# emonosuke/emoASR

Measured on AMD Instinct MI355X. Metric: train frames/sec + decode RTF, Conformer-CTC 23M, 80-mel, 1/2/4/8 GPU, higher is better.
Workload: dtype bf16; 1 GPU; CTC(Conformer) 23M `L2`, bf16, SpecAugment on-GPU, synthetic LibriSpeech-shaped batches (2000 utts, lognormal lengths, ASRBatchSampler packing 30000 frames/50 utts per GPU), one step = accum_grad 5 micro-batches (the reference's accum_grad: 5, asr/train_asr.py:106-128, stacked through the engine in one pass) fwd+bwd, then all-reduce+clip+Adam; dropout 0.1; accum_grad=5, stacked_micro_batches=True, parallelism=dp1

## Files before the change

emoasr_amd/csrc/ctc.hip:

```cpp
#include <algorithm>
#include "common.h"
#include "../../include/emoasr_hip.h"

namespace {

__device__ __forceinline__ float lat_add(float a, float b) {
  const float m = fmaxf(a, b);
  if (m == -INFINITY) return -INFINITY;
  return m + __logf(1.f + __expf(-fabsf(a - b)));
}
__device__ __forceinline__ float lat_add3(float a, float b, float c) {
  const float m = fmaxf(a, fmaxf(b, c));
  if (m == -INFINITY) return -INFINITY;
  return m + __logf(__expf(a - m) + __expf(b - m) + __expf(c - m));
}

template <typename T>
__global__ __launch_bounds__(256) void row_lse_kernel(int V, const T* __restrict__ logits, long ld,
                                                      float* __restrict__ lse, int aligned) {
  __shared__ float red[16];
  const T* row = logits + (long)blockIdx.x * ld;
  constexpr int VEC = 16 / sizeof(T);
  float m = -INFINITY, s = 0.f;
  const int nv = aligned ? V / VEC : 0;
  for (int i = threadIdx.x; i < nv; i += 256) {
    const Vec16<T> v = load16(row + (long)i * VEC);
    float lm = v.get(0);
#pragma unroll
    for (int j = 1; j < VEC; ++j) lm = fmaxf(lm, v.get(j));
    if (lm > m) { s *= __expf(m - lm); m = lm; }
    if (m == -INFINITY) continue;
#pragma unroll
    for (int j = 0; j < VEC; ++j) s += __expf(v.get(j) - m);
  }
  for (int i = nv * VEC + threadIdx.x; i < V; i += 256) {
    const float x = to_f32(row[i]);
    if (x > m) { s *= __expf(m - x); m = x; }
    if (m != -INFINITY) s += __expf(x - m);
  }
  const float gm = block_max(m, red);
  const float gs = block_sum(m == -INFINITY ? 0.f : s * __expf(m - gm), red);
  if (threadIdx.x == 0) lse[blockIdx.x] = gm + logf(gs);
}

__device__ __forceinline__ int ext_label(const int* lab, int s, int blank) {
  return (s & 1) ? lab[s >> 1] : blank;
}

struct UttRows { const long* row0; const int* tpad; const float* uscale; };

template <typename T>
__global__ __launch_bounds__(256) void ctc_gather_kernel(int Tn, int S, int Lmax, const T* __restrict__ logits,
                                                         long ld, const float* __restrict__ lse,
// ... 109 lines not shown
                                                       T* __restrict__ grad, long ldg, const UttRows ur, int aligned) {
  extern __shared__ float rowbuf[];
  const int b = blockIdx.y, t = blockIdx.x;
  if (ur.tpad && t >= ur.tpad[b]) return;
  const long row = (long)b * Tn + t;
  const long lrow = ur.row0 ? ur.row0[b] + t : row;
  T* g = grad + lrow * ldg;
  const float nl = nll[b];
  const bool vec = aligned && (V % 8 == 0) && (ld % 8 == 0) && (ldg % 8 == 0);
  if (t >= elens[b] || !isfinite(nl)) {
    if (vec) {
      float z[8] = {0.f, 0.f, 0.f, 0.f, 0.f, 0.f, 0.f, 0.f};
      for (int v = threadIdx.x * 8; v < V; v += 2048) store8<T>(g + v, z);
    } else {
      for (int v = threadIdx.x; v < V; v += 256) g[v] = from_f32<T>(0.f);
    }
    return;
  }
  const float l = lse[lrow];
  const T* lg = logits + lrow * ld;
  if (vec) {
    for (int v = threadIdx.x * 8; v < V; v += 2048) {
      float x[8];
      load8<T>(lg + v, x);
#pragma unroll
      for (int e = 0; e < 8; ++e) rowbuf[v + e] = __expf(x[e] - l);
    }
  } else {
    for (int v = threadIdx.x; v < V; v += 256) rowbuf[v] = __expf(to_f32(lg[v]) - l);
  }
  __syncthreads();
  const int Sb = 2 * ylens[b] + 1;
  const int* lab = labels + (long)b * Lmax;
  for (int s = threadIdx.x; s < Sb; s += 256) {
    const long o = row * S + s;
    const float occ = __expf(alpha[o] + beta[o] - lp[o] + nl);
    if (occ > 0.f) atomicAdd(&rowbuf[ext_label(lab, s, blank)], -occ);
  }
  __syncthreads();
  const float gs = (gscale_dev ? gscale * gscale_dev[0] : gscale) * (ur.uscale ? ur.uscale[b] : 1.f);
  if (vec) {
    for (int v = threadIdx.x * 8; v < V; v += 2048) {
      float x[8];
#pragma unroll
      for (int e = 0; e < 8; ++e) x[e] = rowbuf[v + e] * gs;
      store8<T>(g + v, x);
    }
  } else {
    for (int v = threadIdx.x; v < V; v += 256) g[v] = from_f32<T>(rowbuf[v] * gs);
  }
}

template <typename T>
__global__ __launch_bounds__(256) void argmax_kernel(int V, const T* __restrict__ logits, long ld,
                                                     int* __restrict__ best) {
  __shared__ float rv[4];
  __shared__ int ri[4];
  const T* row = logits + (long)blockIdx.x * ld;
  float m = -INFINITY; int mi = 0x7fffffff;
  for (int v = threadIdx.x; v < V; v += 256) {
    const float x = to_f32(row[v]);
    if (x > m || (x == m && v < mi)) { m = x; mi = v; }
  }
#pragma unroll
  for (int o = 32; o > 0; o >>= 1) {
    const float om = __shfl_xor(m, o, 64);
    const int oi = __shfl_xor(mi, o, 64);
    if (om > m || (om == m && oi < mi)) { m = om; mi = oi; }
  }
  if ((threadIdx.x & 63) == 0) { rv[threadIdx.x >> 6] = m; ri[threadIdx.x >> 6] = mi; }
  __syncthreads();
  if (threadIdx.x == 0) {
    for (int w = 1; w < 4; ++w)
      if (rv[w] > m || (rv[w] == m && ri[w] < mi)) { m = rv[w]; mi = ri[w]; }
    best[blockIdx.x] = mi == 0x7fffffff ? 0 : mi;
  }
}

__global__ __launch_bounds__(64) void collapse_kernel(int B, int Tn, const int* __restrict__ best, const int* __restrict__ elens,
                                                      int blank, int* __restrict__ hyp, int* __restrict__ hyplen) {
  const int b = blockIdx.x, lane = threadIdx.x;
  if (b >= B) return;
  const int len = min(elens[b], Tn);
  int n = 0, carry = -1;
  for (int t0 = 0; t0 < len; t0 += 64) {
    const int t = t0 + lane;
    const int v = t < len ? best[(long)b * Tn + t] : blank;
    int prev = __shfl_up(v, 1, 64);
    if (lane == 0) prev = carry;
    const bool keep = t < len && v != prev && v != blank;
    const unsigned long long mask = __ballot(keep);
    if (keep) hyp[(long)b * Tn + n + __popcll(mask & ((1ull << lane) - 1ull))] = v;
    n += __popcll(mask);
    carry = __shfl(v, 63, 64);
  }
  if (lane == 0) hyplen[b] = n;
}

}

extern "C" int emoasr_row_lse(int dtype, int M, int V, const void* logits, long ld, float* lse,
                              void* stream) {
  if (M == 0) return 0;
  const int vec = dtype == EMO_BF16 ? 8 : 4;
  const int aligned = (ld % vec == 0) && (((uintptr_t)logits & 15) == 0);
  EMO_DISPATCH(dtype, (row_lse_kernel<T><<<M, 256, 0, (hipStream_t)stream>>>(V, (const T*)logits, ld, lse,
// ... 13 lines not shown
extern "C" int emoasr_ctc_forward_rows(int dtype, int B, int Tn, int V, int Lmax, const void* logits, long ld,
                                       const float* lse, const int* labels, const int* elens, const int* ylens,
                                       int blank, const long* row0, float* lp, float* alpha, float* beta, float* nll,
                                       void* stream) {
  const int S = 2 * Lmax + 1;
  const UttRows ur{row0, nullptr, nullptr};
  EMO_CHECK(S <= 1024, "ctc: 2*Lmax+1=%d exceeds 1024 lattice states", S);
  if (B == 0 || Tn == 0) return 0;
  hipStream_t s = (hipStream_t)stream;
  dim3 ggrid(Tn, B);
  const int gthreads = std::min(256, cdiv(S, 64) * 64);
  EMO_DISPATCH(dtype, (ctc_gather_kernel<T><<<ggrid, gthreads, 0, s>>>(Tn, S, Lmax, (const T*)logits, ld, lse,
                                                                      labels, elens, ylens, blank, lp, ur)));
  const int threads = cdiv(S, 64) * 64;
  ctc_lattice_kernel<<<2 * B, threads, sizeof(float) * 2 * (S + 4), s>>>(B, Tn, S, Lmax, lp, labels, elens,
                                                                        ylens, blank, alpha, beta, nll);
  EMO_LAUNCH_CHECK();
  return 0;
}

extern "C" int emoasr_ctc_grad(int dtype, int B, int Tn, int V, int Lmax, const void* logits, long ld,
                               const float* lse, const int* labels, const int* elens, const int* ylens,
                               int blank, const float* lp, const float* alpha, const float* beta,
                               const float* nll, float gscale, const float* gscale_dev, void* grad, long ldg,
                               void* stream) {
  return emoasr_ctc_grad_rows(dtype, B, Tn, V, Lmax, logits, ld, lse, labels, elens, ylens, blank, lp, alpha, beta, nll, gscale,
                              gscale_dev, nullptr, nullptr, nullptr, grad, ldg, stream);
}

extern "C" int emoasr_ctc_grad_rows(int dtype, int B, int Tn, int V, int Lmax, const void* logits, long ld,
                                    const float* lse, const int* labels, const int* elens, const int* ylens,
                                    int blank, const float* lp, const float* alpha, const float* beta,
                                    const float* nll, float gscale, const float* gscale_dev, const long* row0, const int* tpad,
                                    const float* uscale, void* grad, long ldg, void* stream) {
  const int S = 2 * Lmax + 1;
  EMO_CHECK((row0 != nullptr) == (tpad != nullptr), "ctc_grad_rows: row0 and tpad go together");
  const UttRows ur{row0, tpad, uscale};
  EMO_CHECK((size_t)V * 4 <= 160 * 1024 - 256, "ctc_grad: V=%d too large for an LDS row", V);
  if (B == 0 || Tn == 0) return 0;
  dim3 grid(Tn, B);
  const int aligned = (((uintptr_t)logits | (uintptr_t)grad) & 15) == 0;
  EMO_DISPATCH(dtype, {
    if ((size_t)V * 4 > 64 * 1024)
      hipFuncSetAttribute((const void*)ctc_grad_kernel<T>, hipFuncAttributeMaxDynamicSharedMemorySize, V * 4);
    ctc_grad_kernel<T><<<grid, 256, sizeof(float) * V, (hipStream_t)stream>>>(
        Tn, V, S, Lmax, (const T*)logits, ld, lse, labels, elens, ylens, blank, lp, alpha, beta, nll, gscale,
        gscale_dev,
        (T*)grad, ldg, ur, aligned);
  });
  EMO_LAUNCH_CHECK();
  return 0;
}

extern "C" int emoasr_ctc_greedy(int dtype, int B, int Tn, int V, const void* logits, long ld,
                                 const int* elens, int blank, int* best, int* hyp, int* hyplen,
                                 void* stream) {
  if (B == 0 || Tn == 0) return 0;
  hipStream_t s = (hipStream_t)stream;
  EMO_DISPATCH(dtype, (argmax_kernel<T><<<B * Tn, 256, 0, s>>>(V, (const T*)logits, ld, best)));
  collapse_kernel<<<B, 64, 0, s>>>(B, Tn, best, elens, blank, hyp, hyplen);
  EMO_LAUNCH_CHECK();
  return 0;
}
```

emoasr_amd/engine/encoder.py:

```python
import math
import os

import torch

from .. import ops
from ..ops import ACT_RELU, ACT_SWISH
from .arena import AttnStash, ConvStash, FFNStash, LayerRecord, ParamArena, _Stash, _cfg, h2d_i32, h2d_pack, sinusoid
from .las import LASDecoder
from .rnn_encoder import RNNEncoder
from .rnnt import RNNTDecoder
from .transformer_decoder import TransformerDecoder


class CTCEngine(TransformerDecoder, RNNTDecoder, RNNEncoder, LASDecoder):

    def __init__(self, cfg, module, compute_dtype=torch.bfloat16, bn_buffers=None, f32_split=False, arena=None):
        self.cfg = cfg
        self.split = bool(f32_split) and compute_dtype == torch.float32
        self.d = cfg.enc_hidden_size
        self.h = _cfg(cfg, "enc_num_attention_heads", 0)
        self.nl = cfg.enc_num_layers
        self.conformer = cfg.encoder_type == "conformer"
        self.rnn_enc = cfg.encoder_type == "rnn"
        self.rel = _cfg(cfg, "pos_encode_type", "abs") == "rel"
# ... 467 lines not shown

    def encoder_backward_stacked(self, st, deouts):
        self._defer_wgrads = self._group_wgrads
        try:
            with self._scope():
                self._encoder_bwd_stacked(st, deouts)
        finally:
            self._defer_wgrads = False
            self._wq = []
            self._ln_deferred = []

    def _ctc_train_stacked(self, batches, blank, scales, head):
        A = self.arena
        n = len(batches)
        scales = [1.0 / n] * n if scales is None else [float(v) for v in scales]
        dev = batches[0][0].device
        segs_h, rows_h = [], [0]
        for xs, _, _, _ in batches:
            Bk, Tk, Fd = xs.shape
            T1 = (Tk - 3) // 2 + 1
            segs_h.append((Bk, (T1 - 3) // 2 + 1))
            rows_h.append(rows_h[-1] + Bk * segs_h[-1][1])
        elens_h = [((int(v) - 1) // 2 - 1) // 2 for b in batches for v in b[1]]
        ylens_all = [int(v) for _, _, _, yl in batches for v in yl]
        Lmax = max(max(ylens_all), 1)
        lab = torch.zeros(sum(b for b, _ in segs_h), Lmax, dtype=torch.int32)
        row0, tpad, uscale, b0 = [], [], [], 0
        segw = torch.zeros(n, sum(b for b, _ in segs_h), dtype=torch.float32)
        for k, (_, _, ys, ylens) in enumerate(batches):
            B, T2 = segs_h[k]
            yk = torch.as_tensor(ys)[:, :Lmax].to(torch.int32)
            lab[b0:b0 + B, : yk.shape[1]] = yk
            row0 += [rows_h[k] + b * T2 for b in range(B)]
            tpad += [T2] * B
            uscale += [scales[k] / B] * B
            segw[k, b0:b0 + B] = 1.0 / B
            b0 += B
        elens_d, labels, yl, row0_d, tpad_d, uscale_d, segw_d = h2d_pack(
            [torch.tensor(elens_h, dtype=torch.int32), lab, torch.tensor(ylens_all, dtype=torch.int32),
             torch.tensor(row0, dtype=torch.int64), torch.tensor(tpad, dtype=torch.int32),
             torch.tensor(uscale, dtype=torch.float32), segw], dev)
        eouts, st = self._encoder_fwd_stacked([b[0] for b in batches], [b[1] for b in batches], elens_dev=elens_d)
        segs, rows, elens, Btot, Tmax = st.segs, st.rows, st.elens, st.Btot, st.Tmax
        assert list(segs) == segs_h and list(rows) == rows_h
        w = A.w(head + ".weight")
        V = w.shape[0]
        assert V % 8 == 0, "ctc_train_stacked: vocabulary must be a multiple of 8"
        logits, lse = ops.gemm_nt_lse(eouts, w, A.p(head + ".bias"))
        Vp = (V + 63) // 64 * 64
        dlp = torch.empty(logits.shape[0], Vp, device=dev, dtype=logits.dtype)
        if Vp > V:
            dlp[:, V:].zero_()
        dlogits = dlp[:, :V]
        lp, alpha, beta, nll = ops.ctc_forward_rows(logits, lse, labels, elens, yl, blank, row0_d, Tmax)
        losses = (segw_d * torch.nan_to_num(nll, nan=0.0, posinf=0.0, neginf=0.0)).sum(1)
        ops.ctc_grad_rows(logits, lse, labels, elens, yl, blank, lp, alpha, beta, nll, 1.0, row0_d, tpad_d, uscale_d, dlogits)
        if self.dtype == torch.bfloat16 and os.environ.get("EMOASR_HEAD_NT", "1") != "0":
            self._wgrad(dlogits, eouts, A.g(head + ".weight", tuple(w.shape)), 1.0, A.g(head + ".bias"), 1.0)
            w_t = torch.zeros(w.shape[1], Vp, device=dev, dtype=w.dtype)
            w_t[:, :V].copy_(w.t())
            deouts = ops.gemm_nt(dlp, w_t)
        else:
            deouts = self._lin_bwd(dlogits, eouts, head + ".weight", head + ".bias")
        if self.grad_hook is not None:
            self._flush_wgrads()
            self.grad_hook(A.offsets[head + ".weight"])
        self._encoder_bwd_stacked(st, deouts)
        return losses

    def _lin_bwd(self, dy, x_in, wname, bname, alpha=1.0, **epi):
        A = self.arena
        w = A.w(wname)
        w2 = w.view(w.shape[0], -1)
        self._wgrad(dy, x_in, A.g(wname, tuple(w2.shape)), alpha, A.g(bname), alpha)
        return ops.gemm_nn(dy, w2, alpha=alpha, **epi)

    def _wgrad(self, dy, x_in, out, alpha=1.0, colsum=None, colsum_scale=1.0):
        if self._defer_wgrads:
            self._wq.append((dy, x_in, out, alpha, colsum, colsum_scale))
        else:
            ops.gemm_tn(dy, x_in, out=out, alpha=alpha, accumulate=True, colsum=colsum, colsum_scale=colsum_scale)

    def _hook_after_layer(self, li):
        if not self._layer_rt.wgrad_side:
            self.grad_hook(self._layer_offset(li))
            return
        self._layer_rt.join_wgrads(keep=1)
        if li + 1 < self.nl:
            self.grad_hook(self._layer_offset(li + 1))

    def _layer_offset(self, li):
        if self._layer_lo is None:
            lo = {}
            for n, o in self.arena.offsets.items():
                if n.startswith("encoder.transformers."):
                    k = int(n.split(".")[2])
                    lo[k] = min(lo.get(k, o), o)
            self._layer_lo = lo
        return self._layer_lo[li]

    def _flush_wgrads(self):
        if not self._wq:
            return
        if self._side_wgrads:
            main = torch.cuda.current_stream()
            if self._side is None:
                self._side = torch.cuda.Stream(device=main.device)
            ev = torch.cuda.Event()
            ev.record(main)
            self._side.wait_event(ev)
            ops.gemm_tn_grouped(self._wq, stream=self._side.cuda_stream)
            self._inflight.append(self._wq)
        else:
# ... 255 lines not shown
```

emoasr_amd/lib.py:

```python
import contextlib
import ctypes
import os
from ctypes import (POINTER, Structure, c_char_p, c_float, c_int, c_long, c_uint64,
                    c_void_p)

_HERE = os.path.dirname(os.path.abspath(__file__))
LIB_PATH = os.environ.get("EMOASR_HIP_LIB") or os.path.join(_HERE, "libemoasr_hip.so")

F32, BF16, F32X3 = 0, 1, 2
ACT_NONE, ACT_RELU, ACT_SWISH, ACT_GELU = 0, 1, 2, 3


class Epilogue(Structure):
    _fields_ = [("bias", c_void_p), ("residual", c_void_p), ("pre_out", c_void_p),
                ("dact_pre", c_void_p), ("alpha", c_float), ("res_scale", c_float),
                ("act", c_int), ("dact", c_int), ("ldr", c_int), ("out_f32", c_int),
                ("drop_p", c_float), ("seed", c_uint64)]


class AttnArgs(Structure):
    _fields_ = [("B", c_int), ("H", c_int), ("DK", c_int), ("Tq", c_int), ("Tk", c_int),
                ("ldq", c_long), ("ldk", c_long), ("ldv", c_long), ("ldo", c_long), ("ldp", c_long),
                ("q", c_void_p), ("k", c_void_p), ("v", c_void_p), ("pos", c_void_p),
                ("bias_u", c_void_p), ("bias_v", c_void_p), ("klens", c_void_p),
# ... 205 lines not shown
    "emoasr_attn_step": [I, I, I, I, P, P, P, P, P, P],
    "emoasr_joint_beam_step": [I, POINTER(JointStep), P, P],
    "emoasr_joint_beam_step_parts": [I, POINTER(JointStep), I, P],
    "emoasr_joint_beam_graph_build": [I, POINTER(JointStep), I, I, P],
    "emoasr_joint_beam_graph_launch": [I, I, P],
    "emoasr_attn_dropmask": [I, POINTER(AttnArgs), P, I, P],
    "emoasr_attn_fwd": [I, POINTER(AttnArgs), P],
    "emoasr_attn_bwd": [I, POINTER(AttnArgs), P],
    "emoasr_attn_bwd_fused": [I, POINTER(AttnArgs), P, ctypes.c_size_t, P],
    "emoasr_glu_fwd": [I, I, I, P, P, P],
    "emoasr_glu_bwd": [I, I, I, P, P, P, P],
    "emoasr_dwconv_fwd": [I, I, I, I, I, P, P, P, P, P],
    "emoasr_dwconv_bwd_x": [I, I, I, I, I, P, P, P, P],
    "emoasr_dwconv_fwd_stats": [I, I, I, I, I, P, P, P, P, P, P],
    "emoasr_bn_stats_finalize": [I, I, I, P, P, P, P, P, F, P, P],
    "emoasr_dwconv_bwd_w": [I, I, I, I, I, P, P, P, P, I, P, P],
    "emoasr_bn_stats": [I, I, I, P, P, P, P, P, F, P],
    "emoasr_bn_swish_fwd": [I, I, I, P, P, P, P, P, F, P, P],
    "emoasr_bn_swish_bwd": [I, I, I, P, P, P, P, P, P, F, P, P, P, P, P],
    "emoasr_glu_dwconv_fwd": [I, I, I, I, I, P, P, P, P, P, P],
    "emoasr_bn_swish_bwd_sums": [I, I, I, P, P, P, P, P, P, F, P, P, P, P, P],
    "emoasr_conv_bwd_fused": [I, I, I, I, I, P, P, P, P, P, P, F, P, P, P, P, P, P, P, P],
    "emoasr_strided_copy": [I, I, P, P, I, I, I, I, L, L, L, L, I, P],
    "emoasr_transpose_cast_batched": [I, I, P, P],
    "emoasr_scale_dropout": [I, L, P, P, F, F, U64, P],
    "emoasr_posenc": [I, I, I, I, P, P, F, F, U64, P, P],
    "emoasr_add": [I, L, P, P, P, P],
    "emoasr_row_lse": [I, I, I, P, L, P, P],
    "emoasr_gemm_nt_lse": [I, I, I, I, P, L, P, L, P, L, P, P, P, P],
    "emoasr_ctc_forward": [I, I, I, I, I, P, L, P, P, P, P, I, P, P, P, P, P],
    "emoasr_ctc_grad": [I, I, I, I, I, P, L, P, P, P, P, I, P, P, P, P, F, P, P, L, P],
    "emoasr_rnnt_greedy": [I, I, I, I, I, I, I, I, I, P, P, P, P, P, P, P, P, P, P, P, P, P, L, P, P, P, P],
    "emoasr_wgrad_side_join": [I, P],
    "emoasr_rnnt_beam_lstm": [I, I, I, I, P, L, P, P, P, P, P, P, P, P, P, P, I, P],
    "emoasr_rnnt_beam_joint": [I, I, I, I, I, P, P, P, P, P, P, P, P],
    "emoasr_rnnt_beam_pick": [I, I, I, I, I, P, L, P, L, P],
    "emoasr_rnnlm_step": [I, I, I, I, I, I, I, P, P, P, P, P, P, P, P, P, P, P, P, L, I, P, P, L, P],
    "emoasr_las_attend_fwd": [I, POINTER(LasAttend), P],
    "emoasr_las_attend_bwd": [I, POINTER(LasAttend), P],
    "emoasr_las_dropmask": [POINTER(LasAttend), P, P],
    "emoasr_mlm_expand": [I, I, I, P, P, P, I, I, I, I, P, P, P, P, P],
    "emoasr_sample_rows": [I, I, I, P, L, P, P, U64, L, P, P, P, P],
    "emoasr_gumbel_noise": [I, I, U64, L, P, L, P],
    "emoasr_electra_corrupt": [I, I, P, P, P, P, P, P, P, P],
    "emoasr_bce_head_fwd": [I, I, I, P, L, P, P, P, P, P, P, P, P],
    "emoasr_bce_head_bwd": [I, I, I, P, L, P, P, P, P, F, P, P, L, P, P, P],
    "emoasr_ctc_token_conf": [I, I, I, I, P, L, P, P, P, I, P, P, P, P],
    "emoasr_correct_fuse": [I, I, I, I, I, I, P, L, P, P, L, P, L, F, P, P, P],
    "emoasr_edit_align": [I, I, I, I, P, P, P, P, P, I, P, P, P, P, P, P, P, P],
    "emoasr_rescore_grid": [I, I, I, I, P, P, P, P, P, P, P, P, P, P],
    "emoasr_ctc_beam_batch": [I, I, I, I, P, L, P, P, I, I, ctypes.c_double, I, P, P, P, P, P, L, P, P],
    "emoasr_ctc_forward_rows": [I, I, I, I, I, P, L, P, P, P, P, I, P, P, P, P, P, P],
    "emoasr_ctc_grad_rows": [I, I, I, I, I, P, L, P, P, P, P, I, P, P, P, P, F, P, P, P, P, P, L, P],
    "emoasr_ctc_greedy": [I, I, I, I, P, L, P, I, P, P, P, P],
    "emoasr_embed_fwd": [I, I, I, I, P, P, P, F, F, U64, P, P],
    "emoasr_embed_bwd": [I, I, I, P, P, F, F, U64, P, P],
    "emoasr_lsm_loss": [I, I, I, P, L, P, P, F, P, F, P, P, L, P],
    "emoasr_soft_ce": [I, I, I, P, L, P, P, L, P, P, P, P, F, P, F, P, P, L, P],
    "emoasr_ctc_best_path": [I, I, I, P, P, P, P, P, P, I, P, P],
    "emoasr_ctc_label_map": [I, I, P, P, I, I, P, P, P],
    "emoasr_rnnt_best_path": [I, I, I, P, P, P, P, P, P],
    "emoasr_log_softmax": [I, I, I, P, L, P, L, F, P, L, P],
    "emoasr_topk": [I, I, I, P, L, P, L, P, P, P, P],
    "emoasr_ctc_prefix_init": [I, I, P, I, P, P],
    "emoasr_ctc_prefix_score": [I, I, I, I, P, P, I, P, P, P, P, P, P, I, I, P, P, P],
    "emoasr_lstm_cell_fwd": [I, I, I, P, P, P, L, P, P, P],
    "emoasr_lstm_cell_bwd": [I, I, I, P, L, P, P, P, P, P, P, P],
    "emoasr_lstm_seq_fwd": [I, I, I, I, P, P, P, P, P, P, P, P],
    "emoasr_lstm_seq_bwd": [I, I, I, I, P, P, P, P, P, P, P, L, P],
    "emoasr_bilstm_cell_fwd": [I, I, I, I, I, P, P, L, P, P, P, P, P, P, P, P],
    "emoasr_bilstm_cell_bwd": [I, I, I, I, I, P, P, P, P, P, P, P, P, P],
    "emoasr_bilstm_out": [I, I, I, I, P, P, P, P, F, U64, P],
    "emoasr_bilstm_seq_fwd": [I, I, I, I, P, P, L, P, P, P, P, P, P, P],
    "emoasr_bilstm_seq_bwd": [I, I, I, I, P, P, P, P, P, P, P, P, L, P],
    "emoasr_joint_tanh": [I, I, I, I, I, P, P, P, P],
    "emoasr_joint_reduce": [I, I, I, I, I, P, P, P, P],
    "emoasr_rnnt_forward": [I, I, I, I, I, I, P, P, P, P, I, P, P, P, P, P, P, P],
    "emoasr_rnnt_grad": [I, I, I, I, I, I, P, P, P, P, P, P, P, P, P, P, I, F, P, P, P],
    "emoasr_rnnt_head_fwd": [I, L, I, I, I, I, I, I, P, P, P, P, P, I, P, L, P, P, P, P],
    "emoasr_rnnt_ycol": [I, I, I, I, P, P, P, P],
    "emoasr_rnnt_forward_parts": [I, I, I, I, P, P, P, P, P, P, P, P, P, P],
    "emoasr_rnnt_coef": [I, I, I, I, P, P, P, P, P, P, P, P, P, F, P, P, P, P],
    "emoasr_rnnt_head_grad": [I, I, I, I, P, P, P, P, P, I, P, L, P],
    "emoasr_ce_head_fwd": [I, I, I, I, P, P, P, P, P, P, P, P, P, P, P, P],
    "emoasr_ce_head_sample_fwd": [I, I, I, I, P, P, P, P, P, P, P, P, P, P, P, U64, L, P, P],
    "emoasr_ce_head_grad": [I, I, I, I, P, P, P, P, P, P, F, P, P, P, L, P],
    "emoasr_act_bwd": [I, L, I, P, P, P, P],
    "emoasr_argmax_rows": [I, I, I, P, L, P, P],
    "emoasr_first_not_equal": [I, P, I, P, P],
    "emoasr_sqnorm": [L, P, P, P],
    "emoasr_adam_step": [L, P, P, P, P, F, F, F, F, F, I, P, F, F, P],
    "emoasr_adam_step_ex": [L, P, P, P, P, F, F, F, F, F, I, P, F, F, P, P],
    "emoasr_adamw_step": [L, P, P, P, P, F, F, F, F, I, P, F, F, P, P, P, I, P],
    "emoasr_specaug_apply": [I, I, I, P, P, I, I, P, P, P],
    "emoasr_fbank": [P, L, I, I, I, I, F, P, P, P, I, P],
    "emoasr_cmvn": [I, I, P, P, P, P],
}


class EmoasrHipError(RuntimeError):
    pass


_lib = None


# ... 164 lines not shown
```

emoasr_amd/ops.py:

```python
import ctypes
from ctypes import byref, c_void_p

import os
import threading

import torch

from . import lib
from .lib import ACT_GELU, ACT_NONE, ACT_RELU, ACT_SWISH, BF16, F32, F32X3, AttnArgs, Epilogue

_DT = {torch.float32: F32, torch.bfloat16: BF16}


def dt(t):
    if t.dtype == torch.float32 and split_products():
        return F32X3
    return _DT[t.dtype]


def _p(t):
    return None if t is None else c_void_p(t.data_ptr())


_STREAM_CACHE = None
# ... 592 lines not shown
    B, T, V = logits.shape
    Lmax = labels.shape[1]
    S = 2 * Lmax + 1
    dev = logits.device
    lp = torch.empty(B, T, S, device=dev, dtype=torch.float32)
    alpha = torch.empty(B, T, S, device=dev, dtype=torch.float32)
    beta = torch.empty(B, T, S, device=dev, dtype=torch.float32)
    nll = torch.empty(B, device=dev, dtype=torch.float32)
    lib.call("emoasr_ctc_forward", dt(logits), B, T, V, Lmax, _p(logits), logits.stride(1), _p(lse), _p(labels),
             _p(elens), _p(ylens), blank, _p(lp), _p(alpha), _p(beta), _p(nll), _stream())
    return lp, alpha, beta, nll


def ctc_grad(logits, lse, labels, elens, ylens, blank, lp, alpha, beta, nll, gscale, gscale_dev=None, out=None):
    B, T, V = logits.shape
    ld = logits.stride(1)
    if out is not None:
        assert out.shape == logits.shape and out.dtype == logits.dtype and out.stride(2) == 1
        grad = out
    else:
        grad = torch.empty_like(logits) if ld == V else torch.empty(B, T, ld, device=logits.device, dtype=logits.dtype)[..., :V]
    lib.call("emoasr_ctc_grad", dt(logits), B, T, V, labels.shape[1], _p(logits), logits.stride(1), _p(lse),
             _p(labels), _p(elens), _p(ylens), blank, _p(lp), _p(alpha), _p(beta), _p(nll), gscale, _p(gscale_dev),
             _p(grad),
             grad.stride(1), _stream())
    return grad


def ctc_forward_rows(logits2, lse, labels, elens, ylens, blank, row0, Tmax):
    M, V = logits2.shape
    B, Lmax = labels.shape
    S = 2 * Lmax + 1
    dev = logits2.device
    lp = torch.empty(B, Tmax, S, device=dev, dtype=torch.float32)
    alpha = torch.empty(B, Tmax, S, device=dev, dtype=torch.float32)
    beta = torch.empty(B, Tmax, S, device=dev, dtype=torch.float32)
    nll = torch.empty(B, device=dev, dtype=torch.float32)
    assert row0.dtype == torch.int64
    lib.call("emoasr_ctc_forward_rows", dt(logits2), B, Tmax, V, Lmax, _p(logits2), logits2.stride(0), _p(lse), _p(labels),
             _p(elens), _p(ylens), blank, _p(row0), _p(lp), _p(alpha), _p(beta), _p(nll), _stream())
    return lp, alpha, beta, nll


def ctc_grad_rows(logits2, lse, labels, elens, ylens, blank, lp, alpha, beta, nll, gscale, row0, tpad, uscale, out):
    M, V = logits2.shape
    B, Tmax, _ = lp.shape
    assert out.shape == logits2.shape and out.dtype == logits2.dtype and tpad.dtype == torch.int32 and uscale.dtype == torch.float32
    lib.call("emoasr_ctc_grad_rows", dt(logits2), B, Tmax, V, labels.shape[1], _p(logits2), logits2.stride(0), _p(lse), _p(labels),
             _p(elens), _p(ylens), blank, _p(lp), _p(alpha), _p(beta), _p(nll), gscale, None, _p(row0), _p(tpad), _p(uscale),
             _p(out), out.stride(0), _stream())
    return out


def ctc_greedy(logits, elens, blank):
    B, T, V = logits.shape
    dev = logits.device
    buf = torch.empty(2 * B * T + B, device=dev, dtype=torch.int32)
    best, hyp, hyplen = buf[:B * T].view(B, T), buf[B * T:2 * B * T].view(B, T), buf[2 * B * T:]
    lib.call("emoasr_ctc_greedy", dt(logits), B, T, V, _p(logits), logits.stride(1), _p(elens), blank, _p(best),
             _p(hyp), _p(hyplen), _stream())
    return best, hyp, hyplen


def embed_fwd(ids, table, pe, scale, drop_p=0.0, seed=0):
    B, L = ids.shape
    d = table.shape[1]
    out = torch.empty(B, L, d, device=table.device, dtype=table.dtype)
    lib.call("emoasr_embed_fwd", dt(table), B * L, L, d, _p(ids), _p(table), _p(pe), scale, drop_p, seed, _p(out),
             _stream())
    return out


def embed_bwd(ids, dout, scale, dtable, drop_p=0.0, seed=0):
    B, L = ids.shape
    lib.call("emoasr_embed_bwd", dt(dout), B * L, dout.shape[-1], _p(ids), _p(dout), scale, drop_p, seed,
             _p(_chk(dtable, torch.float32)), _stream())


def lsm_loss(logits, labels, w, lsm_prob, want_grad=False, gscale=1.0, gscale_dev=None, grad=None):
    M, V, ld = _rows(_chk(logits))
    loss = torch.empty(M, device=logits.device, dtype=torch.float32)
    if grad is not None:
        assert want_grad and _chk(grad, logits.dtype).shape == logits.shape and grad.stride(1) == 1
    else:
        grad = torch.empty_like(logits) if want_grad else None
    lib.call("emoasr_lsm_loss", dt(logits), M, V, _p(logits), ld, _p(labels), _p(w), lsm_prob, _p(loss), gscale,
             _p(gscale_dev), _p(grad), 0 if grad is None else grad.stride(0), _stream())
    return loss, grad


def mlm_expand(ys, ylens, row0, r_begin, r_count, Np, mask_id, pad_id=0, total=None, out=None):
    B, N = _chk(ys, torch.int32).shape
    assert ys.is_contiguous() and ylens.numel() == B and row0.numel() == B + 1
    _chk(ylens, torch.int32), _chk(row0, torch.int32)
    assert r_begin >= 0 and r_count >= 1 and (total is None or r_begin + r_count <= total), (r_begin, r_count, total)
    if out is None:
        dev = ys.device
        out = (torch.empty(r_count, Np, device=dev, dtype=torch.int32),) + tuple(
            torch.empty(r_count, device=dev, dtype=torch.int32) for _ in range(3))
    ids, klens, idx, labels = out
    for t in out:
        assert _chk(t, torch.int32).is_contiguous() and t.shape[0] >= r_count
    assert ids.shape[1] == Np
    lib.call("emoasr_mlm_expand", B, N, Np, _p(ys), _p(ylens), _p(row0), r_begin, r_count, mask_id, pad_id, _p(ids), _p(klens),
             _p(idx), _p(labels), _stream())
    return ids[:r_count], klens[:r_count], idx[:r_count], labels[:r_count]
# ... 760 lines not shown
```

include/emoasr_hip.h:

```cpp
#ifndef EMOASR_HIP_H
#define EMOASR_HIP_H
#include <stddef.h>
#include <stdint.h>
#ifdef __cplusplus
extern "C" {
#endif

enum { EMOASR_F32 = 0, EMOASR_BF16 = 1, EMOASR_F32X3 = 2 };
enum { EMOASR_ACT_NONE = 0, EMOASR_ACT_RELU = 1, EMOASR_ACT_SWISH = 2,
       EMOASR_DACT_MUL = 6 };
#define EMOASR_ACT_SAVE_DACT 0x100

const char* emoasr_last_error(void);
int emoasr_version(void);
int emoasr_set_option(const char* name, int value);
int emoasr_get_option(const char* name, int* value, int* default_value);
int emoasr_option_count(void);
const char* emoasr_option_name(int index);
int emoasr_timer_read(const char* name, int* calls, double* ms, int reset);
int emoasr_timer_read_ex(const char* name, int* calls, double* ms, double* flops, double* bytes, int reset);

typedef struct {
  const float* bias;
  const void* residual;
// ... 145 lines not shown
int emoasr_dwconv_bwd_w(int dtype, int B, int T, int C, int K, const void* dy, const void* x, float* dw,
                        float* dbias, int accumulate, float* scratch, void* stream);
long emoasr_dwconv_bwd_w_scratch_floats(int B, int T, int C, int K);
int emoasr_bn_stats(int dtype, int M, int C, const void* y, float* mean, float* var,
                    float* running_mean, float* running_var, float momentum, void* stream);
int emoasr_bn_swish_fwd(int dtype, int M, int C, const void* y, const float* mean, const float* var,
                        const float* gamma, const float* beta, float eps, void* z, void* stream);
long emoasr_bn_swish_bwd_scratch_floats(int M, int C);
int emoasr_bn_swish_bwd(int dtype, int M, int C, const void* dz, const void* y, const float* mean,
                        const float* var, const float* gamma, const float* beta, float eps, void* dy,
                        float* dgamma, float* dbeta, float* scratch, void* stream);
int emoasr_glu_dwconv_fwd(int dtype, int B, int Tn, int C, int K, const void* g, const float* w, const float* bias, void* c,
                          float* part, void* stream);
int emoasr_bn_swish_bwd_sums(int dtype, int M, int C, const void* dz, const void* y, const float* mean, const float* var,
                             const float* gamma, const float* beta, float eps, float* dgamma, float* dbeta, float* scratch,
                             float** tot_out, void* stream);
int emoasr_conv_bwd_fused(int dtype, int B, int Tn, int C, int K, const void* ds, const void* cv, const float* mean,
                          const float* var, const float* gamma, const float* beta, float eps, const float* tot, const void* g,
                          const float* w, void* dg, float* dw, float* dbias, float* scratch, void* stream);

int emoasr_strided_copy(int dtype_in, int dtype_out, const void* in, void* out, int d0, int d1, int d2,
                        int d3, long s0, long s1, long s2, long s3, int accumulate, void* stream);
int emoasr_scale_dropout(int dtype, long n, const void* x, void* y, float scale, float drop_p,
                         uint64_t seed, void* stream);
int emoasr_posenc(int dtype, int B, int T, int N, const void* x, const float* pe, float scale,
                  float drop_p, uint64_t seed, void* y, void* stream);
int emoasr_act_bwd(int dtype, long n, int act, const void* dy, const void* pre, void* dx, void* stream);
int emoasr_add(int dtype, long n, const void* a, const void* b, void* y, void* stream);

typedef struct emoasr_tc_item {
  const float* src; void* dst;
  int rows, cols; long ld_dst;
} emoasr_tc_item_t;
#define EMOASR_TC_MAX 64
int emoasr_transpose_cast_batched(int dtype_out, int n, const emoasr_tc_item_t* items, void* stream);

int emoasr_row_lse(int dtype, int M, int V, const void* logits, long ld, float* lse, void* stream);
int emoasr_gemm_nt_lse(int dtype, int M, int N, int K, const void* A, long lda, const void* B, long ldb, void* C, long ldc,
                       const float* bias, float* part, float* lse, void* stream);
int emoasr_ctc_forward(int dtype, int B, int T, int V, int Lmax, const void* logits, long ld,
                       const float* lse, const int* labels, const int* elens, const int* ylens, int blank,
                       float* lp, float* alpha, float* beta, float* nll, void* stream);
int emoasr_ctc_grad(int dtype, int B, int T, int V, int Lmax, const void* logits, long ld,
                    const float* lse, const int* labels, const int* elens, const int* ylens, int blank,
                    const float* lp, const float* alpha, const float* beta, const float* nll,
                    float gscale, const float* gscale_dev, void* grad, long ldg, void* stream);
int emoasr_ctc_forward_rows(int dtype, int B, int Tn, int V, int Lmax, const void* logits, long ld, const float* lse,
                            const int* labels, const int* elens, const int* ylens, int blank, const long* row0, float* lp,
                            float* alpha, float* beta, float* nll, void* stream);
int emoasr_ctc_grad_rows(int dtype, int B, int Tn, int V, int Lmax, const void* logits, long ld, const float* lse,
                         const int* labels, const int* elens, const int* ylens, int blank, const float* lp, const float* alpha,
                         const float* beta, const float* nll, float gscale, const float* gscale_dev, const long* row0,
                         const int* tpad, const float* uscale, void* grad, long ldg, void* stream);
int emoasr_ctc_greedy(int dtype, int B, int T, int V, const void* logits, long ld, const int* elens,
                      int blank, int* best, int* hyp, int* hyplen, void* stream);

int emoasr_embed_fwd(int dtype, int M, int L, int d, const int* ids, const void* table, const float* pe,
                     float scale, float drop_p, uint64_t seed, void* out, void* stream);
int emoasr_embed_bwd(int dtype, int M, int d, const int* ids, const void* dout, float scale, float drop_p,
                     uint64_t seed, float* dtable, void* stream);
int emoasr_lsm_loss(int dtype, int M, int V, const void* logits, long ld, const int* labels, const float* w,
                    float lsm_prob, float* loss, float gscale, const float* gscale_dev, void* grad, long ldg,
                    void* stream);

int emoasr_soft_ce(int dtype, int R, int V, const void* logits, long ld, const int* lrow, const float* soft, long lds,
                   const int* src, const int* hard, const float* w_soft, const float* w_hard, float lsm_prob,
                   float* loss, float gscale, const float* gscale_dev, void* grad, long ldg, void* stream);
int emoasr_ctc_best_path(int B, int Tn, int Lmax, const float* lp, const float* alpha, const float* beta,
                         const int* labels, const int* elens, const int* ylens, int blank, int* aligns, void* stream);
int emoasr_ctc_label_map(int B, int Tn, const int* aligns, const int* xlens, int blank, int position, int* label_map,
                         int* count, void* stream);

int emoasr_rnnt_best_path(int B, int Tn, int U, const float* alpha, const float* beta, const int* elens,
                          const int* ylens, int* aligns, void* stream);

int emoasr_log_softmax(int dtype, int M, int V, const void* x, long ldx, const float* add, long lda, float mu,
                       float* out, long ldo, void* stream);
int emoasr_topk(int M, int V, int k, const float* x, long ldx, const float* aux, long ldaux, float* vals,
                int* idx, float* aux_out, void* stream);
int emoasr_beam_scores_topk(int dtype, int M, int V, int k, const void* dec, long ldd, const float* lm, long ldl, float mu,
                            float* vals, int* idx, float* lm_at, void* stream);
int emoasr_ctc_prefix_init(int T, int V, const float* x, int blank, float* r, void* stream);
int emoasr_ctc_prefix_score(int nb, int T, int V, int cw, const float* x, const float* prev_states, int cw_prev,
                            const int* parent, const int* pcand, const float* init_state, const int* last,
                            const int* out_len, const int* cands, int blank, int eos, float* log_psi,
                            float* states, void* stream);

int emoasr_lstm_cell_fwd(int dtype, int B, int H, const void* gates_pre, const float* c_prev, void* h, long ldh,
                         float* c, void* gates_act, void* stream);
int emoasr_lstm_cell_bwd(int dtype, int B, int H, const void* dh_out, long lddh, const void* dh_rec, float* dc,
                         const void* gates_act, const float* c_prev, const float* c, void* dgates_pre,
                         void* stream);
int emoasr_lstm_seq_supported(int dtype, int B, int H);
int emoasr_lstm_seq_fwd(int dtype, int U, int B, int H, const void* pre, const void* w_hh, const void* h0, const float* c0,
                        void* hseq, float* cseq, void* gact, void* stream);
long emoasr_lstm_seq_bwd_ws_bytes(int B, int H);
int emoasr_lstm_seq_bwd(int dtype, int U, int B, int H, const void* dh_seq, const void* gact, const float* cseq, const float* c0,
                        const void* w_hh, void* dgp, void* ws, long ws_bytes, void* stream);
long emoasr_lstm_coop_status(void);
int emoasr_bilstm_cell_fwd(int dtype, int B, int T, int H, int s, const int* elens, const void* pre, long ldp, const void* rec,
                           void* hstate, float* cstate, void* hseq, void* hprev, float* cseq, void* gact, void* stream);
int emoasr_bilstm_cell_bwd(int dtype, int B, int T, int H, int s, const int* elens, const void* dy, const void* dh_rec,
                           float* dcstate, const void* gact, const float* cseq, void* dg, void* dgc, void* stream);
int emoasr_bilstm_out(int dtype, int B, int T, int H, const int* elens, const void* x0, const void* x1, void* y, float drop_p,
                      uint64_t seed, void* stream);
int emoasr_bilstm_seq_supported(int dtype, int B, int H);
// ... 325 lines not shown
```

Before: 6.184 million frames/s.

## Split CTC gradient into dense softmax pass overlapped with lattice forward plus sparse fix

The CTC gradient is split into two kernels. A dense kernel writes softmax(logits)*scale for every row, and it runs on a side stream at the same time as the alpha/beta lattice forward. A sparse fix kernel then subtracts occupancies only at label and blank columns, writing a value only where the bf16 result differs. This removes the serialized full-vocabulary pass that followed the forward and replaces LDS atomics with per-label accumulation. The cost is extra stream and event management, a different handling of repeated labels, and possible small numerical differences.

Result: no change. 6.199 million frames/s (median of 5 runs) (+0.2%).

```diff
diff --git a/emoasr_amd/csrc/ctc.hip b/emoasr_amd/csrc/ctc.hip
--- a/emoasr_amd/csrc/ctc.hip
+++ b/emoasr_amd/csrc/ctc.hip
@@ -1,4 +1,7 @@
 #include <algorithm>
+#include <map>
+#include <mutex>
+#include <utility>
 #include "common.h"
 #include "../../include/emoasr_hip.h"
 
@@ -214,6 +217,132 @@
 }
 
 template <typename T>
+__global__ __launch_bounds__(256) void ctc_grad_dense_kernel(int Tn, int V, const T* __restrict__ logits, long ld,
+                                                             const float* __restrict__ lse, const int* __restrict__ elens,
+                                                             float gscale, const float* __restrict__ gscale_dev,
+                                                             T* __restrict__ grad, long ldg, const UttRows ur, int aligned) {
+  const int b = blockIdx.y, t = blockIdx.x;
+  if (ur.tpad && t >= ur.tpad[b]) return;
+  const long lrow = ur.row0 ? ur.row0[b] + t : (long)b * Tn + t;
+  T* g = grad + lrow * ldg;
+  const bool vec = aligned && (V % 8 == 0) && (ld % 8 == 0) && (ldg % 8 == 0);
+  if (t >= elens[b]) {
+    if (vec) {
+      float z[8] = {0.f, 0.f, 0.f, 0.f, 0.f, 0.f, 0.f, 0.f};
+      for (int v = threadIdx.x * 8; v < V; v += 2048) store8<T>(g + v, z);
+    } else {
+      for (int v = threadIdx.x; v < V; v += 256) g[v] = from_f32<T>(0.f);
+    }
+    return;
+  }
+  const float l = lse[lrow];
+  const T* lg = logits + lrow * ld;
+  const float gs = (gscale_dev ? gscale * gscale_dev[0] : gscale) * (ur.uscale ? ur.uscale[b] : 1.f);
+  if (vec) {
+    for (int v = threadIdx.x * 8; v < V; v += 2048) {
+      float x[8];
+      load8<T>(lg + v, x);
+#pragma unroll
+      for (int e = 0; e < 8; ++e) x[e] = __expf(x[e] - l) * gs;
+      store8<T>(g + v, x);
+    }
+  } else {
+    for (int v = threadIdx.x; v < V; v += 256) g[v] = from_f32<T>(__expf(to_f32(lg[v]) - l) * gs);
+  }
+}
+
+constexpr int CTC_FIX_FR = 16;
+template <typename T>
+__device__ __forceinline__ void fix_store(T* g, float v, float p, float gs) {
+  const T nv = from_f32<T>(v * gs), dv = from_f32<T>(p * gs);
+  if constexpr (sizeof(T) == 2) {
+    if (__builtin_bit_cast(unsigned short, nv) != __builtin_bit_cast(unsigned short, dv)) *g = nv;
+  } else {
+    if (__builtin_bit_cast(unsigned, nv) != __builtin_bit_cast(unsigned, dv)) *g = nv;
+  }
+}
+template <typename T>
+__global__ __launch_bounds__(256) void ctc_grad_fix_kernel(int Tn, int V, int S, int Lmax, const int* __restrict__ labels,
+                                                           const int* __restrict__ elens, const int* __restrict__ ylens,
+                                                           int blank, const float* __restrict__ lp,
+                                                           const float* __restrict__ alpha, const float* __restrict__ beta,
+                                                           const float* __restrict__ nll, float gscale,
+                                                           const float* __restrict__ gscale_dev, T* __restrict__ grad, long ldg,
+                                                           const UttRows ur, int aligned) {
+  extern __shared__ float fixbuf[];
+  const int b = blockIdx.y, t0 = blockIdx.x * CTC_FIX_FR;
+  int tend = min(elens[b], Tn);
+  if (ur.tpad) tend = min(tend, ur.tpad[b]);
+  if (t0 >= tend) return;
+  const int nf = min(CTC_FIX_FR, tend - t0);
+  const long lrow0 = (ur.row0 ? ur.row0[b] : (long)b * Tn) + t0;
+  const long row0 = (long)b * Tn + t0;
+  const float nl = nll[b];
+  if (!isfinite(nl)) {
+    const bool vec = aligned && (V % 8 == 0) && (ldg % 8 == 0);
+    for (int f = 0; f < nf; ++f) {
+      T* g = grad + (lrow0 + f) * ldg;
+      if (vec) {
+        float z[8] = {0.f, 0.f, 0.f, 0.f, 0.f, 0.f, 0.f, 0.f};
+        for (int v = threadIdx.x * 8; v < V; v += 2048) store8<T>(g + v, z);
+      } else {
+        for (int v = threadIdx.x; v < V; v += 256) g[v] = from_f32<T>(0.f);
+      }
+    }
+    return;
+  }
+  float* occ = fixbuf;
+  int* lab = (int*)(fixbuf + 8 * S);
+  int* nxt = lab + Lmax;
+  int* fst = nxt + Lmax;
+  const int L = min(ylens[b], Lmax), Sb = 2 * L + 1;
+  for (int i = threadIdx.x; i < L; i += 256) lab[i] = labels[(long)b * Lmax + i];
+  __syncthreads();
+  for (int i = threadIdx.x; i < L; i += 256) {
+    const int c = lab[i];
+    int n = -1, first = 1;
+    for (int j = L - 1; j > i; --j) n = lab[j] == c ? j : n;
+    for (int j = 0; j < i; ++j) first = lab[j] == c ? 0 : first;
+    nxt[i] = n;
+    fst[i] = first;
+  }
+  const float gs = (gscale_dev ? gscale * gscale_dev[0] : gscale) * (ur.uscale ? ur.uscale[b] : 1.f);
+  const int w = threadIdx.x >> 6, lane = threadIdx.x & 63;
+  for (int k = 0; k < CTC_FIX_FR / 4; ++k) {
+    const int f = k * 4 + w;
+    const bool live = f < nf;
+    float* oc = occ + (long)((k & 1) * 4 + w) * S;
+    const float* lpr = lp + (row0 + f) * S;
+    if (live) {
+      const float* ar = alpha + (row0 + f) * S;
+      const float* br = beta + (row0 + f) * S;
+      for (int s = lane; s < Sb; s += 64) {
+        const float v = __expf(ar[s] + br[s] - lpr[s] + nl);
+        oc[s] = v > 0.f ? v : 0.f;
+      }
+    }
+    __syncthreads();
+    if (!live) continue;
+    T* g = grad + (lrow0 + f) * ldg;
+    for (int s = 2 * lane + 1; s < Sb; s += 128) {
+      const int i = s >> 1, c = lab[i];
+      if (c == blank || !fst[i] || (unsigned)c >= (unsigned)V) continue;
+      const float p = __expf(lpr[s]);
+      float v = p - oc[s];
+      for (int j = nxt[i]; j >= 0; j = nxt[j]) v -= oc[2 * j + 1];
+      fix_store(g + c, v, p, gs);
+    }
+    if (lane == 63 && (unsigned)blank < (unsigned)V) {
+      const float p = __expf(lpr[0]);
+      float v = p;
+      for (int s = 0; s < Sb; ++s)
+        if (!(s & 1) || lab[s >> 1] == blank) v -= oc[s];
+      fix_store(g + blank, v, p, gs);
+    }
+  }
+}
+
+template <typename T>
 __global__ __launch_bounds__(256) void argmax_kernel(int V, const T* __restrict__ logits, long ld,
                                                      int* __restrict__ best) {
   __shared__ float rv[4];
@@ -333,6 +462,91 @@
   return 0;
 }
 
+namespace {
+
+struct CtcSide {
+  hipStream_t side = nullptr;
+  hipEvent_t fork = nullptr, done = nullptr;
+  int mode = -1;
+};
+std::mutex g_ctc_mu;
+std::map<std::pair<int, hipStream_t>, CtcSide> g_ctc;
+
+CtcSide* ctc_side_of(hipStream_t s, bool with_stream) {
+  int dev = 0;
+  if (hipGetDevice(&dev) != hipSuccess) return nullptr;
+  CtcSide& c = g_ctc[{dev, s}];
+  if (with_stream && !c.side) {
+    hipStream_t st = nullptr;
+    hipError_t e = hipStreamCreateWithFlags(&st, hipStreamNonBlocking);
+    if (e != hipSuccess) return nullptr;
+    if (hipEventCreateWithFlags(&c.fork, hipEventDisableTiming) != hipSuccess ||
+        hipEventCreateWithFlags(&c.done, hipEventDisableTiming) != hipSuccess) {
+      hipStreamDestroy(st);
+      return nullptr;
+    }
+    c.side = st;
+  }
+  return &c;
+}
+
+}
+
+extern "C" int emoasr_ctc_loss_grad_rows(int dtype, int B, int Tn, int V, int Lmax, const void* logits, long ld, const float* lse,
+                                         const int* labels, const int* elens, const int* ylens, int blank, const long* row0,
+                                         const int* tpad, const float* uscale, float gscale, const float* gscale_dev, float* lp,
+                                         float* alpha, float* beta, float* nll, void* grad, long ldg, void* stream) {
+  const int S = 2 * Lmax + 1;
+  EMO_CHECK((row0 != nullptr) == (tpad != nullptr), "ctc_loss_grad_rows: row0 and tpad go together");
+  EMO_CHECK(S <= 1024, "ctc: 2*Lmax+1=%d exceeds 1024 lattice states", S);
+  EMO_CHECK(dtype == EMO_F32 || dtype == EMO_F32X3 || dtype == EMO_BF16, "bad dtype %d", dtype);
+  if (B == 0 || Tn == 0) return 0;
+  hipStream_t s = (hipStream_t)stream;
+  const UttRows ur{row0, tpad, uscale};
+  dim3 grid(Tn, B);
+  const int aligned = (((uintptr_t)logits | (uintptr_t)grad) & 15) == 0;
+  hipStreamCaptureStatus cap = hipStreamCaptureStatusNone;
+  const bool capturing = hipStreamIsCapturing(s, &cap) != hipSuccess || cap != hipStreamCaptureStatusNone;
+  std::lock_guard<std::mutex> lk(g_ctc_mu);
+  CtcSide* c = ctc_side_of(s, !capturing);
+  EMO_CHECK(c != nullptr, "ctc_loss_grad_rows: no side stream");
+  const bool side = !capturing;
+  hipStream_t ds = side ? c->side : s;
+  if (side) {
+    EMO_CHECK(hipEventRecord(c->fork, s) == hipSuccess && hipStreamWaitEvent(c->side, c->fork, 0) == hipSuccess,
+              "ctc_loss_grad_rows: fork failed");
+  }
+  EMO_DISPATCH(dtype, (ctc_grad_dense_kernel<T><<<grid, 256, 0, ds>>>(Tn, V, (const T*)logits, ld, lse, elens, gscale, gscale_dev,
+                                                                      (T*)grad, ldg, ur, aligned)));
+  hipError_t le = hipGetLastError();
+  if (side) {
+    EMO_CHECK(hipEventRecord(c->done, c->side) == hipSuccess, "ctc_loss_grad_rows: hipEventRecord failed");
+  }
+  int rc = le == hipSuccess ? emoasr_ctc_forward_rows(dtype, B, Tn, V, Lmax, logits, ld, lse, labels, elens, ylens, blank, row0, lp,
+                                                      alpha, beta, nll, stream)
+                            : 2;
+  if (side) {
+    EMO_CHECK(hipStreamWaitEvent(s, c->done, 0) == hipSuccess, "ctc_loss_grad_rows: join failed");
+  }
+  c->mode = side ? 1 : 0;
+  if (le != hipSuccess) emo_set_error("%s:%d launch failed: %s", __FILE__, __LINE__, hipGetErrorString(le));
+  if (rc) return rc;
+  dim3 fgrid(cdiv(Tn, CTC_FIX_FR), B);
+  EMO_DISPATCH(dtype, (ctc_grad_fix_kernel<T><<<fgrid, 256, sizeof(float) * (8 * S + 3 * Lmax), s>>>(
+                          Tn, V, S, Lmax, labels, elens, ylens, blank, lp, alpha, beta, nll, gscale, gscale_dev, (T*)grad, ldg, ur,
+                          aligned)));
+  EMO_LAUNCH_CHECK();
+  return 0;
+}
+
+extern "C" int emoasr_ctc_loss_grad_mode(void* stream) {
+  std::lock_guard<std::mutex> lk(g_ctc_mu);
+  int dev = 0;
+  if (hipGetDevice(&dev) != hipSuccess) return -1;
+  auto it = g_ctc.find({dev, (hipStream_t)stream});
+  return it == g_ctc.end() ? -1 : it->second.mode;
+}
+
 extern "C" int emoasr_ctc_greedy(int dtype, int B, int Tn, int V, const void* logits, long ld,
                                  const int* elens, int blank, int* best, int* hyp, int* hyplen,
                                  void* stream) {
diff --git a/emoasr_amd/engine/encoder.py b/emoasr_amd/engine/encoder.py
--- a/emoasr_amd/engine/encoder.py
+++ b/emoasr_amd/engine/encoder.py
@@ -543,13 +543,25 @@
         if Vp > V:
             dlp[:, V:].zero_()
         dlogits = dlp[:, :V]
-        lp, alpha, beta, nll = ops.ctc_forward_rows(logits, lse, labels, elens, yl, blank, row0_d, Tmax)
+        head_nt = self.dtype == torch.bfloat16 and os.environ.get("EMOASR_HEAD_NT", "1") != "0"
+        overlap = os.environ.get("EMOASR_CTC_OVERLAP", "1") != "0"
+        w_t = None
+        if overlap:
+            if head_nt:
+                w_t = torch.zeros(w.shape[1], Vp, device=dev, dtype=w.dtype)
+                w_t[:, :V].copy_(w.t())
+            lp, alpha, beta, nll, _ = ops.ctc_loss_grad_rows(logits, lse, labels, elens, yl, blank, 1.0, dlogits, row0=row0_d,
+                                                             tpad=tpad_d, uscale=uscale_d, Tmax=Tmax)
+        else:
+            lp, alpha, beta, nll = ops.ctc_forward_rows(logits, lse, labels, elens, yl, blank, row0_d, Tmax)
         losses = (segw_d * torch.nan_to_num(nll, nan=0.0, posinf=0.0, neginf=0.0)).sum(1)
-        ops.ctc_grad_rows(logits, lse, labels, elens, yl, blank, lp, alpha, beta, nll, 1.0, row0_d, tpad_d, uscale_d, dlogits)
-        if self.dtype == torch.bfloat16 and os.environ.get("EMOASR_HEAD_NT", "1") != "0":
+        if not overlap:
+            ops.ctc_grad_rows(logits, lse, labels, elens, yl, blank, lp, alpha, beta, nll, 1.0, row0_d, tpad_d, uscale_d, dlogits)
+        if head_nt:
             self._wgrad(dlogits, eouts, A.g(head + ".weight", tuple(w.shape)), 1.0, A.g(head + ".bias"), 1.0)
-            w_t = torch.zeros(w.shape[1], Vp, device=dev, dtype=w.dtype)
-            w_t[:, :V].copy_(w.t())
+            if w_t is None:
+                w_t = torch.zeros(w.shape[1], Vp, device=dev, dtype=w.dtype)
+                w_t[:, :V].copy_(w.t())
             deouts = ops.gemm_nt(dlp, w_t)
         else:
             deouts = self._lin_bwd(dlogits, eouts, head + ".weight", head + ".bias")
diff --git a/emoasr_amd/lib.py b/emoasr_amd/lib.py
--- a/emoasr_amd/lib.py
+++ b/emoasr_amd/lib.py
@@ -281,6 +281,8 @@
     "emoasr_ctc_beam_batch": [I, I, I, I, P, L, P, P, I, I, ctypes.c_double, I, P, P, P, P, P, L, P, P],
     "emoasr_ctc_forward_rows": [I, I, I, I, I, P, L, P, P, P, P, I, P, P, P, P, P, P],
     "emoasr_ctc_grad_rows": [I, I, I, I, I, P, L, P, P, P, P, I, P, P, P, P, F, P, P, P, P, P, L, P],
+    "emoasr_ctc_loss_grad_rows": [I, I, I, I, I, P, L, P, P, P, P, I, P, P, P, F, P, P, P, P, P, P, L, P],
+    "emoasr_ctc_loss_grad_mode": [P],
     "emoasr_ctc_greedy": [I, I, I, I, P, L, P, I, P, P, P, P],
     "emoasr_embed_fwd": [I, I, I, I, P, P, P, F, F, U64, P, P],
     "emoasr_embed_bwd": [I, I, I, P, P, F, F, U64, P, P],
diff --git a/emoasr_amd/ops.py b/emoasr_amd/ops.py
--- a/emoasr_amd/ops.py
+++ b/emoasr_amd/ops.py
@@ -668,6 +668,35 @@
     return out
 
 
+def ctc_loss_grad_rows(logits, lse, labels, elens, ylens, blank, gscale, out, row0=None, tpad=None, uscale=None, Tmax=None,
+                       gscale_dev=None):
+    stacked = row0 is not None
+    if stacked:
+        M, V = logits.shape
+        assert row0.dtype == torch.int64 and tpad.dtype == torch.int32 and (uscale is None or uscale.dtype == torch.float32)
+        ld, ldg = logits.stride(0), out.stride(0)
+    else:
+        B_, Tmax, V = logits.shape
+        assert tpad is None
+        ld, ldg = logits.stride(1), out.stride(1)
+    assert out.shape == logits.shape and out.dtype == logits.dtype and out.stride(-1) == 1 and logits.stride(-1) == 1
+    B, Lmax = labels.shape
+    S = 2 * Lmax + 1
+    dev = logits.device
+    lp = torch.empty(B, Tmax, S, device=dev, dtype=torch.float32)
+    alpha = torch.empty(B, Tmax, S, device=dev, dtype=torch.float32)
+    beta = torch.empty(B, Tmax, S, device=dev, dtype=torch.float32)
+    nll = torch.empty(B, device=dev, dtype=torch.float32)
+    lib.call("emoasr_ctc_loss_grad_rows", dt(logits), B, Tmax, V, Lmax, _p(logits), ld, _p(lse), _p(labels), _p(elens), _p(ylens),
+             blank, _p(row0), _p(tpad), _p(uscale), gscale, _p(gscale_dev), _p(lp), _p(alpha), _p(beta), _p(nll), _p(out), ldg,
+             _stream())
+    return lp, alpha, beta, nll, out
+
+
+def ctc_loss_grad_mode():
+    return int(lib.load().emoasr_ctc_loss_grad_mode(_stream()))
+
+
 def ctc_greedy(logits, elens, blank):
     B, T, V = logits.shape
     dev = logits.device
diff --git a/include/emoasr_hip.h b/include/emoasr_hip.h
--- a/include/emoasr_hip.h
+++ b/include/emoasr_hip.h
@@ -221,6 +221,11 @@
                          const int* labels, const int* elens, const int* ylens, int blank, const float* lp, const float* alpha,
                          const float* beta, const float* nll, float gscale, const float* gscale_dev, const long* row0,
                          const int* tpad, const float* uscale, void* grad, long ldg, void* stream);
+int emoasr_ctc_loss_grad_rows(int dtype, int B, int Tn, int V, int Lmax, const void* logits, long ld, const float* lse,
+                              const int* labels, const int* elens, const int* ylens, int blank, const long* row0,
+                              const int* tpad, const float* uscale, float gscale, const float* gscale_dev, float* lp,
+                              float* alpha, float* beta, float* nll, void* grad, long ldg, void* stream);
+int emoasr_ctc_loss_grad_mode(void* stream);
 int emoasr_ctc_greedy(int dtype, int B, int T, int V, const void* logits, long ld, const int* elens,
                       int blank, int* best, int* hyp, int* hyplen, void* stream);
 
```
